# SamStudio8/gretel

Hardware: AMD Instinct MI355X
Metric: haplotypes/sec + SNP-edge-evals/sec on 10k-SNP synthetic contig (higher is better)
Workload: dtype f32 counts / f64 log-likelihoods

## Files before the change

gretel_amd/csrc/gretel_hip.hip:

```cpp

#include <hip/hip_runtime.h>

#include <algorithm>
#include <cmath>
#include <cstdarg>
#include <cstdio>
#include <cstdlib>
#include <cstring>
#include <atomic>
#include <chrono>
#include <map>
#include <mutex>
#include <new>
#include <string>
#include <thread>
#include <vector>

#include "gretel_hip.h"
#include "gh_detlog.h"


static thread_local char g_err[512] = "";

static int fail(int code, const char *fmt, ...)
// ... 1133 lines not shown
        return;
    }
    hipLaunchKernelGGL((k_scan<LC, false>), dim3(G1), dim3(SEG_THREADS), lds_scan, stream, P);
    hipLaunchKernelGGL((k_emit<LC>), dim3(S), dim3(SEG_THREADS), lds_emit, stream, P);
}

static int launch_seg_walk(gh_handle *h, uint8_t *d_path, double *d_lmsel, int rearm, int check_masks)
{
    int rc = alloc_seg(h);
    if (rc) return rc;
    seg_params P;
    P.N = h->N; P.L = h->L; P.rearm = rearm; P.check_masks = check_masks;
    P.G = h->lt; P.minfo = h->minfo; P.rinfo = h->rinfo; P.mt = h->cfg.marginal_term; P.nanp = h->cfg.marginal_term && h->cfg.offer_zero; P.sm = h->sm; P.st = h->dstate;
    P.hist = h->seg_hist; P.maps = h->seg_maps; P.pmaps = h->seg_pmaps; P.gmaps = h->seg_gmaps; P.segmin = h->seg_min;
    P.smin = h->seg_smin; P.gmin = h->seg_gmin; P.cm5snap = h->cm5snap;
    P.rws = 0; P.W = h->W; P.esz = (int)esize(h); P.band = h->band; P.halo = h->rws ? h->seg_halo : nullptr; P.patch_off = 0;
    P.rwflags = reinterpret_cast<int2 *>(h->seg_min + CW_MAX_SEG);
    P.path_out = d_path; P.lmsel = d_lmsel ? d_lmsel : h->lmsel1;
    if (h->L < 1 || h->L > SEG_MAX_L_NARROW) return fail(GH_ERR_STATE, "segment-parallel walk needs L <= %d", SEG_MAX_L_NARROW);
    prof_begin(h, GH_K_WALK);
    switch (h->L) {
        case 1: launch_seg_lc<1>(h, P); break;
        case 2: launch_seg_lc<2>(h, P); break;
        case 3: launch_seg_lc<3>(h, P); break;
        case 4: launch_seg_lc<4>(h, P); break;
        case 5: launch_seg_lc<5>(h, P); break;
        case 6: launch_seg_lc<6>(h, P); break;
    }
    prof_end(h, GH_K_WALK, (double)h->N * ((1.0 + (double)h->L) * CELL * esize(h) + 28.0));
    return post_launch(h, "k_seg/k_scan/k_emit");
}

static size_t rws_lds_bytes(int LC, bool five)
{
    (void)five;
    size_t b = max_cls(LC, [&](int R) { return seg_lds_total(R, LC); });
    if (b < (size_t)SEG_THREADS * 8) b = (size_t)SEG_THREADS * 8;
    return (b + 15) & ~(size_t)15;
}

static size_t rws_patch_off(const gh_handle *h, int LC)
{
    const bool five = seg_radix_ok(5, LC);
    const seg_geom g4 = seg_geometry(h->N, LC, 4), g5 = five ? seg_geometry(h->N, LC, 5) : g4;
    size_t off = rws_lds_bytes(LC, five);
    if (h->cfg.cond_mode == GH_COND_C || h->cfg.cond_mode == GH_COND_E) {
        const int longest = g4.seglen > g5.seglen ? g4.seglen : g5.seglen;
        const size_t need = (size_t)SEG_THREADS * 8 + (size_t)(longest + LC + 1) * NSYM * h->W * NSYM * esize(h);
        if (need > off) off = (need + 15) & ~(size_t)15;
    }
    return off;
}
#define RWS_LDS_MAX (160 * 1024 - 3 * 1024 - 512)

template <typename T, int LC, bool COL>
static void launch_rwseg_lc(gh_handle *h, seg_params P, const rws_params &Q)
{
    constexpr bool five = seg_radix_ok(5, LC);
    const int N = h->N;
    (void)five;
    const int S = (int)max_cls(LC, [&](int R) { return (size_t)seg_geometry(N, LC, R).S; }), G1 = (int)max_cls(LC, [&](int R) { return (size_t)seg_geometry(N, LC, R).G1; });
    const size_t off = rws_patch_off(h, LC);
    const size_t lds = off + sizeof(seg_patch);
    const size_t lds_scan = max_cls(LC, [&](int R) { return scan_lds_bytes(N, LC, R); });
    const size_t lds_emit = max_cls(LC, [&](int R) { return emit_lds_bytes(N, LC, R); });
    static std::atomic<size_t> set_rws[64], set_scan[64], set_emit[64];
    const int dv = h->dev & 63;
    if (lds > set_rws[dv]) { hipFuncSetAttribute((const void *)k_rwseg<T, LC, COL>, hipFuncAttributeMaxDynamicSharedMemorySize, (int)lds); set_rws[dv] = lds; }
    if (lds_scan > set_scan[dv]) { hipFuncSetAttribute((const void *)k_scan<LC, false>, hipFuncAttributeMaxDynamicSharedMemorySize, (int)lds_scan); set_scan[dv] = lds_scan; }
    if (lds_emit > set_emit[dv]) { hipFuncSetAttribute((const void *)k_emit<LC>, hipFuncAttributeMaxDynamicSharedMemorySize, (int)lds_emit); set_emit[dv] = lds_emit; }
    P.patch_off = (int)off;
    P.rws = 1;
    prof_begin(h, GH_K_RWSEG);
    hipLaunchKernelGGL((k_rwseg<T, LC, COL>), dim3(S), dim3(SEG_THREADS), lds, h->stream, P, Q);
    const int wl = h->W < LC ? h->W : LC;
    prof_end(h, GH_K_RWSEG, (double)N * (double)LC * CELL * esize(h) +
             (double)(N + 1) * ((double)h->W * 2.0 * esize(h) + 1.0 + CELL * esize(h) + 2 * 64 + 88 + 8) +
             (double)N * ((double)wl * 7 * esize(h) + (double)LC * LT_ROW * 8.0));
    const size_t lds_small = max_cls(LC, [&](int R) { return emit_small_lds_bytes(N, LC, R); });
    if (lds_small <= 64 * 1024 && !(getenv("GH_EMIT_SMALL") && atoi(getenv("GH_EMIT_SMALL")) == 0)) {
        static std::atomic<size_t> set_small[64];
        if (lds_small > set_small[dv]) { hipFuncSetAttribute((const void *)k_emit_small<LC>, hipFuncAttributeMaxDynamicSharedMemorySize, (int)lds_small); set_small[dv] = lds_small; }
        hipLaunchKernelGGL((k_emit_small<LC>), dim3(S), dim3(SEG_THREADS), lds_small, h->stream, P);
        return;
    }
    hipLaunchKernelGGL((k_scan<LC, false>), dim3(G1), dim3(SEG_THREADS), lds_scan, h->stream, P);
    hipLaunchKernelGGL((k_emit<LC>), dim3(S), dim3(SEG_THREADS), lds_emit, h->stream, P);
}

static int launch_rwseg(gh_handle *h, const uint8_t *d_prev, gh_path_rec *d_prev_rec, int prev_slot, double min_remove,
                        uint8_t *d_path, double *d_lmsel, int check_masks)
{
    int rc = alloc_seg(h);
    if (rc) return rc;
    seg_params P;
    P.N = h->N; P.L = h->L; P.rearm = 1; P.check_masks = check_masks;
    P.G = h->lt; P.minfo = h->minfo; P.rinfo = h->rinfo; P.mt = h->cfg.marginal_term; P.nanp = h->cfg.marginal_term && h->cfg.offer_zero; P.sm = h->sm; P.st = h->dstate;
    P.hist = h->seg_hist; P.maps = h->seg_maps; P.pmaps = h->seg_pmaps; P.gmaps = h->seg_gmaps; P.segmin = h->seg_min;
    P.smin = h->seg_smin; P.gmin = h->seg_gmin; P.cm5snap = h->cm5snap;
    P.rws = 1; P.W = h->W; P.esz = (int)esize(h); P.band = h->band; P.halo = h->seg_halo; P.patch_off = 0;
    P.rwflags = reinterpret_cast<int2 *>(h->seg_min + CW_MAX_SEG);
    P.path_out = d_path; P.lmsel = d_lmsel;
    rws_params Q;
    Q.band = h->band; Q.cnt = h->cnt; Q.marg = h->marg; Q.minfo = h->minfo; Q.rinfo = h->need_rinfo ? h->rinfo : nullptr; Q.G = h->lt;
    Q.nvalid = h->nvalid; Q.cmask = h->cmask; Q.path = d_prev; Q.min_remove = min_remove;
    Q.partial = h->partial + (size_t)prev_slot * h->spin_partial_stride;
    Q.rec = d_prev_rec; Q.cond_mode = h->cfg.cond_mode; Q.offer_zero = h->cfg.offer_zero;
    if (h->L < 1 || h->L > SEG_MAX_L_NARROW) return fail(GH_ERR_STATE, "k_rwseg needs L <= %d", SEG_MAX_L_NARROW);
    prof_begin(h, GH_K_WALK);
    const bool f64 = h->cfg.storage == GH_STORAGE_F64;
    const bool col = h->cfg.cond_mode == GH_COND_C || h->cfg.cond_mode == GH_COND_E;
    switch (h->L) {
#define RWS_CASE(n) case n: if (f64) { if (col) launch_rwseg_lc<double, n, true>(h, P, Q); else launch_rwseg_lc<double, n, false>(h, P, Q); } \
                            else { if (col) launch_rwseg_lc<float, n, true>(h, P, Q); else launch_rwseg_lc<float, n, false>(h, P, Q); } break;
        RWS_CASE(1) RWS_CASE(2) RWS_CASE(3) RWS_CASE(4) RWS_CASE(5) RWS_CASE(6)
#undef RWS_CASE
// ... 711 lines not shown
    *n_out = 0; *hole_at = 0;
    if (max_paths == 0) return GH_OK;
    int rc;
    if (!h->have_orig && (rc = gh_snapshot_original(h))) return rc;
    const size_t n1 = (size_t)h->N + 1;
    if ((rc = ensure_spin_buffers(h, max_paths))) return rc;
    uint8_t *d_paths = h->spin_paths;
    gh_path_rec *d_recs = h->spin_recs;
    hipError_t e = hipSuccess;
    rc = GH_OK;
    bool seg = seg_ok(h->wmode, h->L);
    h->seg6 = false;
    if (rc == GH_OK && !seg && h->wmode == WM_SEG && h->L == SEG_MAX_L_NARROW && !(getenv("GH_SEG6") && atoi(getenv("GH_SEG6")) == 0)) {
        rc = ensure_lt(h);
        dev_state look;
        if (rc == GH_OK) {
            e = hipMemcpyAsync(&look, h->dstate, sizeof look, hipMemcpyDeviceToHost, h->stream);
            if (e == hipSuccess) e = hipStreamSynchronize(h->stream);
            if (e != hipSuccess) rc = fail(GH_ERR_HIP, "gh_spin failed: %s", hipGetErrorString(e));
            else if (look.ranked) { seg = true; h->seg6 = true; }
        }
    }
    h->fuse = false;
    if (rc == GH_OK && seg && h->need_rinfo && h->W <= RW_FUSE_HALO && rw_lanes(h) == 8 && getenv("GH_FUSE") && atoi(getenv("GH_FUSE")) >= 1) {
        rc = ensure_lt(h);
        dev_state look;
        if (rc == GH_OK) {
            e = hipMemcpyAsync(&look, h->dstate, sizeof look, hipMemcpyDeviceToHost, h->stream);
            if (e == hipSuccess) e = hipStreamSynchronize(h->stream);
            if (e != hipSuccess) rc = fail(GH_ERR_HIP, "gh_spin failed: %s", hipGetErrorString(e));
            else {
                const int R = look.ranked ? 4 : 5;
                const int ppb = 256 / rw_lanes(h);
                const bool small = emit_small_lds_bytes(h->N, h->L, R) <= 64 * 1024 && !(getenv("GH_EMIT_SMALL") && atoi(getenv("GH_EMIT_SMALL")) == 0);
                const bool force = getenv("GH_FUSE") && atoi(getenv("GH_FUSE")) == 2;
                if ((!small || force) && seg_radix_ok(R, h->L) && rw_fuse_lds_bytes(h->N, h->L, R, ppb, h->W) <= 64 * 1024 && (rc = alloc_seg(h)) == GH_OK) {
                    h->fuse = true;
                    h->fuse_lds = rw_fuse_lds_bytes(h->N, h->L, R, ppb, h->W);
                    if (hipMemsetAsync(&h->dstate->maxstates, 0, sizeof(int), h->stream) != hipSuccess) rc = fail(GH_ERR_HIP, "gh_spin failed: hipMemsetAsync");
                }
            }
        }
    }
    h->rws = false;
    int rws_S = 0;
    if (rc == GH_OK && seg && !h->fuse && !h->lt_full && rw_lanes(h) == 8 &&
        !(getenv("GH_RWSEG") && atoi(getenv("GH_RWSEG")) == 0)) {
        const bool five = seg_radix_ok(5, h->L);
        const seg_geom g4 = seg_geometry(h->N, h->L, 4), g5 = five ? seg_geometry(h->N, h->L, 5) : g4;
        const bool small = (five ? max2(emit_small_lds_bytes(h->N, h->L, 4), emit_small_lds_bytes(h->N, h->L, 5)) : emit_small_lds_bytes(h->N, h->L, 4)) <= 64 * 1024 &&
                           !(getenv("GH_EMIT_SMALL") && atoi(getenv("GH_EMIT_SMALL")) == 0);
        const int longest = g4.seglen > g5.seglen ? g4.seglen : g5.seglen;
        const bool small_ok = !(getenv("GH_RWSEG_SMALL") && atoi(getenv("GH_RWSEG_SMALL")) == 0);
        if ((!small || small_ok) && longest + h->L + 1 <= SEG_THREADS / 8 && rws_patch_off(h, h->L) + sizeof(seg_patch) <= RWS_LDS_MAX &&
            (rc = alloc_seg(h)) == GH_OK) {
            rws_S = g4.S > g5.S ? g4.S : g5.S;
            const size_t need = (size_t)rws_S * h->L * NSYM * h->W * NSYM * esize(h);
            if (need > h->seg_halo_bytes) {
                if ((e = hipStreamSynchronize(h->stream)) != hipSuccess) rc = fail(GH_ERR_HIP, "gh_spin failed: %s", hipGetErrorString(e));
                else {
                    hipFree(h->seg_halo); h->seg_halo = nullptr; h->seg_halo_bytes = 0;
                    if (hipMalloc(&h->seg_halo, need) != hipSuccess) rc = fail(GH_ERR_NOMEM, "hipMalloc failed");
                    else h->seg_halo_bytes = need;
                }
            }
            h->rws = rc == GH_OK;
        }
    }
    int nb = rw_blocks(h, seg || cw_ok(h->wmode, h->L));
    if (h->rws && rws_S > nb) nb = rws_S;
    h->spin_partial_stride = nb;
    if (rc == GH_OK) rc = ensure_partial(h, nb, max_paths > h->spin_cap ? max_paths : h->spin_cap);
    if (rc == GH_OK) rc = reset_spin_state(h, h->rws ? h->partial : nullptr, h->rws ? (size_t)nb * max_paths : 0);
    const bool optimistic = seg && !h->lt_full;
    dev_state hs;
    memset(&hs, 0, sizeof hs);
    int first = 0;
    h->spin_requeues = 0;
    const bool cw = rc == GH_OK && !seg && cw_ok(h->wmode, h->L) && !h->cw_off;
    bool cw_gave_up = false;
    if (cw) {
        spin_io io;
        io.max_paths = max_paths; io.min_remove = min_remove; io.n1 = n1; io.nb = nb;
        io.d_paths = d_paths; io.d_recs = d_recs; io.paths_out = paths_out; io.recs = recs; io.no_reweight = false;
        rc = spin_candidate_pools(h, io, hs, &first, &cw_gave_up);
    }
    while ((!cw || cw_gave_up) && rc == GH_OK) {
        int launched = first;
        for (int s = first; s < max_paths && rc == GH_OK; s++) {
            if (!optimistic || s == first) { if ((rc = ensure_lt(h, !seg))) break; }
            const int cmk = !(optimistic && s > first) ? 0 : (s == h->force_stale_at && h->spin_requeues == 0 ? 2 : 1);
            if (h->rws) {
                if (s == first) rc = launch_walk(h, d_paths + n1 * s, d_recs + s, min_remove, 1, h->spin_lmsel + n1 * s, cmk);
                else rc = launch_rwseg(h, d_paths + n1 * (s - 1), d_recs + (s - 1), s - 1, min_remove, d_paths + n1 * s, h->spin_lmsel + n1 * s, cmk);
                if (rc == GH_OK && s == max_paths - 1)
                    rc = launch_reweight_marg(h, d_paths + n1 * s, min_remove, 1, d_recs + s, s, true, s > first, 0, h->spin_lmsel + n1 * s);
                if (rc) break;
                launched = s + 1;
                continue;
            }
            if ((rc = launch_walk(h, d_paths + n1 * s, d_recs + s, min_remove, 1, h->spin_lmsel + n1 * s, cmk))) break;
            if ((rc = launch_reweight_marg(h, d_paths + n1 * s, seg ? min_remove : 0.0, 1, d_recs + s, s, seg, optimistic && s > first, 0,
                                           h->spin_lmsel + n1 * s))) break;
            launched = s + 1;
        }
        if (rc == GH_OK && launched > 0 && (seg || cw_gave_up)) {
            hipLaunchKernelGGL(k_hp, dim3(launched, 2), dim3(64), 0, h->stream, (const double *)h->spin_lmsel, n1, (const uint8_t *)d_paths, n1,
// ... 1039 lines not shown
```

gretel_amd/csrc/segwalk.hpp:

```cpp
#pragma once

#include "seg_geom.hpp"

struct seg_params {
    int N, L;
    int rearm;
    int check_masks;
    const double *G;
    const double *minfo;
    const double *rinfo;
    int mt;
    int nanp;
    symmap sm;
    dev_state *st;
    uint32_t *hist;
    uint16_t *maps;
    uint16_t *pmaps;
    uint16_t *gmaps;
    double *segmin;
    double *smin;
    double *gmin;
    uint8_t *cm5snap;
    uint8_t *path_out;
    double *lmsel;
// ... 32 lines not shown
    if (first) {
        if (fr.x & 1) st->cm_same = 0;
        if (fr.x & 2) st->nodel = 0;
        if (fr.x & 4) st->narrow = 0;
        if (fr.y < st->first_hole) st->first_hole = fr.y;
    }
    if (P.check_masks == 2 || (P.check_masks && (fr.x & 1))) {
        if (first) st->lt_stale = 1;
        return false;
    }
    if (first) st->cur_hole = fr.y;
    return true;
}

template <int R>
__device__ __forceinline__ unsigned seg_argmax(const double (&vin)[R], bool nanp = false)
{
    static_assert(R == 4 || R == 5, "four ranks or five symbols");
    double v[R];
#pragma unroll
    for (int b = 0; b < R; b++) v[b] = vin[b];
    if (R == 5 && nanp) {
#pragma unroll
        for (int b = 1; b < R; b++) v[b] = v[b] != v[b] ? -INFINITY : v[b];
    }
    const bool c01 = v[1] > v[0], c23 = v[3] > v[2];
    const double m01 = vmax_f64(v[0], v[1]), m23 = vmax_f64(v[2], v[3]);
    const bool c = m23 > m01;
    unsigned idx = c ? (c23 ? 3u : 2u) : (c01 ? 1u : 0u);
    if constexpr (R == 5) {
        const double m = vmax_f64(m01, m23);
        idx = v[4] > m ? 4u : idx;
        idx = v[0] != v[0] ? 0u : idx;
    }
    return idx;
}

__device__ __forceinline__ double vmin_f64(double a, double b)
{
    double r;
    asm("v_min_f64 %0, %1, %2" : "=v"(r) : "v"(a), "v"(b));
    return r;
}

struct seg_patch {
    double row[SEG_MAX_L_NARROW][SEG_MAX_L_NARROW][LT_ROW];
    int row6[SEG_MAX_L_NARROW];
    int col[SEG_MAX_L_NARROW][SEG_MAX_L_NARROW];
    unsigned rmask[SEG_MAX_L_NARROW][SEG_MAX_L_NARROW];
    int colmode;
    double lm4[SEG_MAX_L_NARROW][4], lm5[SEG_MAX_L_NARROW][5];
    uint8_t cmall[SEG_THREADS / 8];
};

template <int R, int LC, bool TRACK, bool NANP = false>
__device__ __forceinline__ void seg_body(const seg_params &P, unsigned char *smem, const seg_patch *patch = nullptr)
{
    typedef typename seg_radix<R>::next_t next_t;
    constexpr int BITS = seg_radix<R>::BITS;
    constexpr unsigned MASK = (1u << BITS) - 1u;
    constexpr unsigned NS = seg_ipow(R, LC), NI = NS / R, RR = R * R;
    constexpr int CH = seg_chunk(R, LC);
    constexpr int SPT = (NS + SEG_THREADS - 1) / SEG_THREADS;
    const seg_geom g = seg_geometry(P.N, LC, R);
    const int s = blockIdx.x, tid = threadIdx.x;
    if (s >= g.S) return;
    const int t0 = s * g.seglen;
    const int t1 = t0 + g.seglen < P.N ? t0 + g.seglen : P.N;
    double *Gs = reinterpret_cast<double *>(smem);
    next_t *Nx = reinterpret_cast<next_t *>(Gs + (size_t)(CH + LC - 1) * LC * RR);
    double *Ms = reinterpret_cast<double *>(smem + seg_lds_bytes(R, LC));
    constexpr bool nanp = NANP;
    double mn[SPT];
#pragma unroll
    for (int q = 0; q < SPT; q++) mn[q] = INFINITY;

    unsigned sigma[SPT];
#pragma unroll
    for (int q = 0; q < SPT; q++) sigma[q] = (unsigned)(tid + q * SEG_THREADS) < NS ? (unsigned)(tid + q * SEG_THREADS) : 0u;

    SEG_STAMP(0);
    for (int c0 = t0; c0 < t1; c0 += CH) {
        const int nc = t1 - c0 < CH ? t1 - c0 : CH;
        const int nsrc = nc + LC - 1;
        for (int e = tid; e < nsrc * LC * R; e += SEG_THREADS) {
            const int d = e % R, l = (e / R) % LC, ii = e / (R * LC);
            const int i = c0 + 1 - LC + ii;
            double v[R];
#pragma unroll
            for (int b = 0; b < R; b++) v[b] = 0.0;
            if (i >= 0) {
                const double *src = P.G + (((size_t)i * 6 + (i == 0 ? 5 : d)) * LC + l) * LT_ROW;
#pragma unroll
                for (int b = 0; b < R; b++) v[b] = src[b];
                if (P.mt && l == 0) {
                    const double *lm = R == 4 ? P.rinfo + (size_t)(i + 1) * RINFO : P.minfo + (size_t)(i + 1) * MINFO;
                    if (patch && c0 == t0 && t0 > 0 && ii + 1 < LC) lm = R == 4 ? patch->lm4[ii + 1] : patch->lm5[ii + 1];
#pragma unroll
                    for (int b = 0; b < R; b++) v[b] = lm[b] + v[b];
                }
            }
            double *dst = Gs + (size_t)e * R;
#pragma unroll
            for (int b = 0; b < R; b++) dst[b] = v[b];
        }
        if (patch && c0 == t0 && t0 > 0) {
            __syncthreads();
            for (int e = tid; e < LC * LC * R; e += SEG_THREADS) {
                const int b = e % R, l = (e / R) % LC, hp = e / (R * LC);
                if (patch->colmode) {
                    const int col = patch->col[hp][l];
                    if (col >= 0 && col < R && ((patch->rmask[hp][l] >> b) & 1u)) {
                        double v = patch->row[hp][l][b];
                        if (P.mt && l == 0) {
                            const int i = t0 + 1 - LC + hp;
                            const double *lm = R == 4 ? P.rinfo + (size_t)(i + 1) * RINFO : P.minfo + (size_t)(i + 1) * MINFO;
                            if (hp + 1 < LC) lm = R == 4 ? patch->lm4[hp + 1] : patch->lm5[hp + 1];
                            v = lm[col] + v;
                        }
                        Gs[((size_t)(hp * LC + l) * R + b) * R + col] = v;
                    }
                    continue;
                }
                const int d = patch->row6[hp];
                if (d >= 0 && d < R) {
                    double v = patch->row[hp][l][b];
                    if (P.mt && l == 0) {
                        const int i = t0 + 1 - LC + hp;
                        const double *lm = R == 4 ? P.rinfo + (size_t)(i + 1) * RINFO : P.minfo + (size_t)(i + 1) * MINFO;
                        if (hp + 1 < LC) lm = R == 4 ? patch->lm4[hp + 1] : patch->lm5[hp + 1];
                        v = lm[b] + v;
                    }
                    Gs[((size_t)(hp * LC + l) * R + d) * R + b] = v;
                }
            }
        }
        if (TRACK) {
            for (int e = tid; e < nc * R; e += SEG_THREADS) {
                const int tl = e / R, b = e - tl * R;
                const int t = c0 + 1 + tl;
                Ms[e] = R == 4 ? P.rinfo[(size_t)t * RINFO + 4 + b] : P.minfo[(size_t)t * MINFO + 5 + b];
            }
        }
        __syncthreads();
        SEG_STAMP(1);
        {
            constexpr int SH = LC >= 4 ? 1 : 0;
            constexpr unsigned NJ = NI / (SH ? R : 1);
            for (unsigned task = tid; task < (unsigned)nc * NJ; task += SEG_THREADS) {
                const unsigned tl = task / NJ, j = task - tl * NJ;
                double xl[R][R];
#pragma unroll
                for (int dL = 0; dL < R; dL++) {
                    const double *row = Gs + ((size_t)(tl * LC + (LC - 1)) * R + dL) * R;
#pragma unroll
                    for (int b = 0; b < R; b++) xl[dL][b] = row[b];
                }
                double acc[R];
                unsigned rem = j;
                constexpr int NYOUNG = LC - 1 - SH;
                if constexpr (NYOUNG >= 1) {
#pragma unroll
                    for (int l = 1; l <= NYOUNG; l++) {
                        const unsigned d = rem % R;
                        rem /= R;
                        const double *row = Gs + ((size_t)((tl + LC - l) * LC + (l - 1)) * R + d) * R;
#pragma unroll
                        for (int b = 0; b < R; b++) acc[b] = l == 1 ? row[b] : acc[b] + row[b];
                    }
                }
#pragma unroll
                for (int dS = 0; dS < (SH ? R : 1); dS++) {
                    double acc2[R];
                    if constexpr (SH) {
                        const double *row = Gs + ((size_t)((tl + 1) * LC + (LC - 2)) * R + dS) * R;
#pragma unroll
                        for (int b = 0; b < R; b++) acc2[b] = NYOUNG >= 1 ? acc[b] + row[b] : row[b];
                    } else {
#pragma unroll
                        for (int b = 0; b < R; b++) acc2[b] = acc[b];
                    }
                    unsigned packed = 0;
#pragma unroll
                    for (int dL = 0; dL < R; dL++) {
                        double v[R];
#pragma unroll
                        for (int b = 0; b < R; b++) v[b] = LC >= 2 ? acc2[b] + xl[dL][b] : xl[dL][b];
                        packed |= seg_argmax<R>(v, nanp) << (BITS * dL);
                    }
                    Nx[(size_t)tl * NI + j + (SH ? dS * NJ : 0)] = (next_t)packed;
                }
            }
        }
        __syncthreads();
        SEG_STAMP(2);
        {
            constexpr int DPW = seg_radix<R>::DPW;
            const int w0 = (c0 - t0) / DPW;
            auto walk_word = [&](int tw, int nu, auto full_) {
                constexpr bool full = decltype(full_)::value;
                unsigned word[SPT];
#pragma unroll
                for (int q = 0; q < SPT; q++) word[q] = 0;
                const next_t *rows = Nx + (size_t)tw * NI;
#pragma unroll
                for (int u = 0; u < DPW; u++) {
                    if (full || u < nu) {
#pragma unroll
                        for (int q = 0; q < SPT; q++) {
                            const unsigned sg = sigma[q];
                            const unsigned hi = sg / NI, idx = sg - hi * NI;
                            const unsigned d = ((unsigned)rows[u * NI + idx] >> (BITS * hi)) & MASK;
                            word[q] |= d << (BITS * u);
                            sigma[q] = idx * R + d;
                            if (TRACK) mn[q] = vmin_f64(mn[q], Ms[(tw + u) * R + d]);
                        }
                    }
                }
#pragma unroll
                for (int q = 0; q < SPT; q++) {
                    const unsigned s0 = tid + q * SEG_THREADS;
                    if (s0 < NS) P.hist[((size_t)s * g.NW + w0 + tw / DPW) * NS + s0] = word[q];
                }
            };
            int tw = 0;
            for (; tw + DPW <= nc; tw += DPW) walk_word(tw, DPW, std::true_type{});
            if (tw < nc) walk_word(tw, nc - tw, std::false_type{});
        }
        SEG_STAMP(3);
        __syncthreads();
    }
#pragma unroll
    for (int q = 0; q < SPT; q++) {
        const unsigned s0 = tid + q * SEG_THREADS;
        if (s0 < NS) {
            P.maps[(size_t)s * NS + s0] = (uint16_t)sigma[q];
            if (TRACK) P.smin[(size_t)s * NS + s0] = mn[q];
        }
    }
    SEG_STAMP(4);
}

#include "segmix.hpp"

template <int LC, bool TRACK>
__global__ void __launch_bounds__(SEG_THREADS) k_seg(seg_params P)
{
    extern __shared__ __align__(16) unsigned char seg_smem[];
    dev_state *st = P.st;
    const dev_ctl c = load_ctl(st);
    if (c.stop || c.lt_stale) return;
    if (P.check_masks == 2 || (P.check_masks && c.cm_same == 0)) {
        if (blockIdx.x == 0 && threadIdx.x == 0) st->lt_stale = 1;
        return;
    }
    if (blockIdx.x == 0 && threadIdx.x == 0) st->cur_hole = c.first_hole;
    const int cls = __builtin_amdgcn_readfirstlane(seg_class(c, LC));
    if (cls == 4) seg_body<4, LC, TRACK>(P, seg_smem);
    else if constexpr (seg_radix_ok(5, LC)) {
        if constexpr (LC == SEGM_L && !TRACK) { if (cls == SEG_CLS_MIXED) { seg_body_mixed<LC, false>(P, seg_smem); return; } }
        if (P.nanp) seg_body<5, LC, TRACK, true>(P, seg_smem);
        else seg_body<5, LC, TRACK, false>(P, seg_smem);
    }
}

template <int R, int LC, bool TRACK>
__device__ __forceinline__ void scan_body(const seg_params &P, unsigned char *smem)
{
    constexpr int NS = seg_ns(R, LC);
    const seg_geom g = seg_geometry(P.N, LC, R);
    const int grp = blockIdx.x, tid = threadIdx.x;
    if (grp >= g.G1) return;
    const int s_lo = grp * g.G2;
    const int n = (s_lo + g.G2 <= g.S ? g.G2 : g.S - s_lo);
    uint16_t *M = reinterpret_cast<uint16_t *>(smem);
    const uint16_t *src = P.maps + (size_t)s_lo * NS;
    if constexpr (NS % 8 == 0) {
        const uint4 *s4 = reinterpret_cast<const uint4 *>(src);
        uint4 *d4 = reinterpret_cast<uint4 *>(M);
        for (int e = tid; e < n * (NS / 8); e += SEG_THREADS) d4[e] = s4[e];
    } else {
        for (int e = tid; e < n * NS; e += SEG_THREADS) M[e] = src[e];
// ... 787 lines not shown
    }
    RW_STAMP(4);
    __shared__ unsigned s_flags;
    __shared__ int s_hole;
    if (tid == 0) { s_flags = 0; s_hole = 0x7fffffff; }
#pragma unroll
    for (int o = 32; o > 0; o >>= 1) removed += __shfl_xor(removed, o);
    if ((tid & 63) == 0) s_sum4[tid >> 6] = removed;
    __syncthreads();
    if (flag_bits) atomicOr(&s_flags, flag_bits);
    if (hole_p != 0x7fffffff) atomicMin(&s_hole, hole_p);
    __syncthreads();
    if (tid == 0) {
        partial[blockIdx.x] = (s_sum4[0] + s_sum4[1]) + (s_sum4[2] + s_sum4[3]);
        const unsigned f = s_flags;
        if (f & 1u) atomicAnd(&st->cm_same, 0);
        if (f & 2u) atomicAnd(&st->nodel, 0);
        if (f & 4u) atomicAnd(&st->narrow, 0);
        if (s_hole != 0x7fffffff) atomicMin(&st->first_hole, s_hole);
    }
    RW_STAMP(5);
}

__device__ __forceinline__ double lane_f64(double v, int lane)
{
    const long long b = __double_as_longlong(v);
    const int lo = __builtin_amdgcn_readlane((int)b, lane), hi = __builtin_amdgcn_readlane((int)(b >> 32), lane);
    return __longlong_as_double(((long long)hi << 32) | (long long)(unsigned)lo);
}
__device__ __forceinline__ double wave_min_f64(double v)
{
    double x;
    x = dpp_f64<0xB1>(v); v = x < v ? x : v;
    x = dpp_f64<0x4E>(v); v = x < v ? x : v;
    x = dpp_f64<0x141>(v); v = x < v ? x : v;
    x = dpp_f64<0x140>(v); v = x < v ? x : v;
    const double r0 = lane_f64(v, 0), r1 = lane_f64(v, 16), r2 = lane_f64(v, 32), r3 = lane_f64(v, 48);
    const double a = r1 < r0 ? r1 : r0, b = r3 < r2 ? r3 : r2;
    return b < a ? b : a;
}

struct rws_params {
    void *band;
    double *cnt, *marg, *minfo, *rinfo, *G;
    int32_t *nvalid;
    uint32_t *cmask;
    const uint8_t *path;
    double min_remove;
    double *partial;
    gh_path_rec *rec;
    int cond_mode, offer_zero;
};

template <typename T, int LC, bool COL>
__device__ __forceinline__ bool rwseg_reweight(const seg_params &P, const rws_params &Q, const dev_ctl &c, unsigned char *smem, seg_patch *patch)
{
    const int N = P.N, W = P.W, L = LC, tid = threadIdx.x, sblk = blockIdx.x;
    const symmap sm = P.sm;
    dev_state *st = P.st;
    double *sred = reinterpret_cast<double *>(smem);
    __shared__ double s_logtab[256];
    logtab_stage(s_logtab);
    if (tid < SEG_MAX_L_NARROW) patch->row6[tid] = -1;
    if (tid < SEG_MAX_L_NARROW * SEG_MAX_L_NARROW) { (&patch->col[0][0])[tid] = -1; (&patch->rmask[0][0])[tid] = 0u; }
    if (tid == 0) patch->colmode = COL ? 1 : 0;
    const int R = seg_class(c, L);
    const seg_geom g = seg_geometry(N, L, R);
    if (sblk >= g.S) { if (tid == 0) { Q.partial[sblk] = 0.0; P.rwflags[sblk] = make_int2(0, 0x7fffffff); } return false; }
    RWS_STAMP(0);
    double vs[7];
#pragma unroll
    for (int k = 0; k < 7; k++) { const int q = (tid & 63) + 64 * k; vs[k] = q < g.S ? P.segmin[q] : INFINITY; }
    const int t0 = sblk * g.seglen;
    const int t1 = t0 + g.seglen < N ? t0 + g.seglen : N;
    const int nh = sblk > 0 ? L : 0;
    const int nown = (t1 - t0) + (sblk == 0 ? 1 : 0);
    const int slot = tid >> 3, s = tid & 7;
    const bool in = slot < nh + nown;
    const bool halo = in && slot < nh;
    const int p = !in ? 0 : (halo ? t0 + 1 - L + slot : (sblk == 0 ? slot : t0 + 1 + (slot - nh)));
    const bool act = in && p <= N;
    const bool own = act && !halo;
    const size_t pos_elems = (size_t)NSYM * W * NSYM;
    T *bandT = static_cast<T *>(Q.band);
    const T *blk = halo ? static_cast<const T *>(P.halo) + ((size_t)sblk * L + slot) * pos_elems : bandT + (size_t)p * pos_elems;
    if (COL) {
        T *blkL = reinterpret_cast<T *>(smem + (size_t)SEG_THREADS * 8);
        const size_t wper = pos_elems * sizeof(T) / 4;
        const uint32_t *srcH = reinterpret_cast<const uint32_t *>(static_cast<const T *>(P.halo) + (size_t)sblk * L * pos_elems);
        const int p_first = sblk == 0 ? 0 : t0 + 1;
        const uint32_t *srcO = reinterpret_cast<const uint32_t *>(bandT + (size_t)p_first * pos_elems);
        uint32_t *dst = reinterpret_cast<uint32_t *>(blkL);
        for (size_t q = tid; q < (size_t)nh * wper; q += SEG_THREADS) dst[q] = srcH[q];
        for (size_t q = tid; q < (size_t)nown * wper; q += SEG_THREADS) dst[(size_t)nh * wper + q] = srcO[q];
        __syncthreads();
        blk = blkL + (size_t)(in ? slot : 0) * pos_elems;
    }
    const int d0 = s + 1, j0 = p + d0;
    int mult0 = 0;
    if (act && d0 <= W) {
        if (j0 <= N - 1) mult0 = (d0 == 1) ? 2 : 1;
        else if (j0 == N) mult0 = (d0 == 1) ? 1 : 0;
        else if (j0 == N + 1) mult0 = (p == N) ? 1 : 0;
    }
    const int a = act ? Q.path[p] : 0;
    const int b0 = mult0 ? ((j0 == N + 1) ? Q.path[0] : Q.path[j0]) : 0;
    const bool lag_row = Q.G && act && p < N && d0 <= L && j0 <= N && (!COL || (mult0 > 0 && d0 <= W));
    T crow[NSYM];
#pragma unroll
    for (int x = 0; x < NSYM; x++) crow[x] = (act && s < NSYM) ? blk[((size_t)s * W) * NSYM + x] : (T)0;
    int nv_t = 0;
    uint32_t cm_t = 0;
    if (lag_row) { nv_t = Q.nvalid[j0]; cm_t = CM_CAND(Q.cmask[j0]); }
    const uint32_t cm_old = (own && s == 7) ? Q.cmask[p] : 0u;
    const bool need_row = act && d0 <= W && (mult0 > 0 || lag_row);
    const size_t roff = ((size_t)a * W + (size_t)((d0 <= W ? d0 : 1) - 1)) * NSYM;
    const size_t run0 = COL ? ((size_t)((d0 <= W ? d0 : 1) - 1)) * NSYM + b0 : roff;
    const size_t rstride = COL ? (size_t)W * NSYM : 1;
    const int esel = COL ? a : b0;
    T rrow[NSYM];
#pragma unroll
    for (int x = 0; x < NSYM; x++) rrow[x] = need_row ? blk[run0 + (size_t)x * rstride] : (T)0;
    double v0 = vs[0];
#pragma unroll
    for (int k = 1; k < 7; k++) v0 = vs[k] < v0 ? vs[k] : v0;
    const double minm = wave_min_f64(v0);
    RWS_STAMP(1);
    static_assert(SEG_MAX_L_NARROW * 8 <= 64 && SEG_MAX_L_NARROW * SEG_MAX_L_NARROW <= 64, "halo lane groups and the patch's arming lanes in one wavefront");
    const double ratio = minm < Q.min_remove ? Q.min_remove : minm;
    if (sblk == 0 && tid == 0) seg_finish(st, Q.rec, N, minm, Q.min_remove);
    RWS_STAMP(2);
    double removed = 0.0;
    int na = -1, nb = -1;
    T nval = (T)0;
    if (mult0) {
        T cur = rrow[0];
#pragma unroll
        for (int x = 1; x < NSYM; x++) cur = (x == esel) ? rrow[x] : cur;
        for (int q = 0; q < mult0; q++) {
            const double old = (double)cur;
            const double nw = old - ratio * old;
            cur = (T)nw;
            if (own) removed += old - nw;
        }
        if (own) bandT[(size_t)p * pos_elems + roff + b0] = cur;
#pragma unroll
        for (int x = 0; x < NSYM; x++) rrow[x] = (x == esel) ? cur : rrow[x];
        if (d0 == 1) { na = a; nb = b0; nval = cur; }
    }
    na = __shfl(na, 0, 8); nb = __shfl(nb, 0, 8);
    nval = (T)__shfl((double)nval, 0, 8);
    __syncthreads();
    unsigned flag_bits = 0;
    int hole_p = 0x7fffffff;
    double cs[NSYM];
    double tot = 0.0;
    int nv = 0;
    uint32_t cm = 0;
    T acc = (T)0;
#pragma unroll
    for (int x = 0; x < NSYM; x++) {
        T v = crow[x];
        if (s == na && x == nb) v = nval;
        acc = acc + v;
    }
    const double mine = (double)acc;
#pragma unroll
    for (int x = 0; x < NSYM; x++) {
        cs[x] = __shfl(mine, x, 8);
        if (cs[x] > 0) {
            tot += cs[x];
            if ((VALID_MASK >> x) & 1) { nv++; cm |= 1u << x; }
        }
    }
    const uint32_t cand = Q.offer_zero ? VALID_MASK : cm;
    const uint32_t cmw = cm | (cand << 8);
    const uint32_t cm5 = cm5_of_cmask(sm, cand);
    if (own) {
        if (s < NSYM) {
// ... 92 lines not shown
        const double nv_i = (double)nv;
        int row6 = a6;
        if (ranked && a6 < 5) row6 = ((cm5 >> a6) & 1u) ? __popc(cm5 & ((1u << a6) - 1u)) : -1;
        if (row6 >= 0) {
            double out[LT_ROW];
            if (!(a6 < 5 || p == 0)) {
#pragma unroll
                for (int q = 0; q < LT_ROW; q++) out[q] = 0.0;
            } else {
                double rowv[NSYM];
                T racc = (T)0;
#pragma unroll
                for (int x = 0; x < NSYM; x++) { rowv[x] = (double)rrow[x]; racc = racc + rrow[x]; }
                const double sum = (double)racc;
                const double den = (Q.cond_mode == GH_COND_A) ? (double)nv_t + sum : (Q.cond_mode == GH_COND_D ? nv_i + sum : nv_i + ca);
                constexpr int VS[LT_ROW] = {0, 1, 2, 3, 5};
                double xq[LT_ROW], v[LT_ROW];
                bool odd = false;
#pragma unroll
                for (int q = 0; q < LT_ROW; q++) xq[q] = (1.0 + rowv[VS[q]]) / den;
#pragma unroll
                for (int q = 0; q < LT_ROW; q++) odd |= !gh_log10_is_normal(xq[q]);
#pragma unroll
                for (int q = 0; q < LT_ROW; q++) v[q] = gh_log10_normal_tab(xq[q], 0, s_logtab, GH_LOG_BOTH);
                if (odd) {
#pragma unroll
                    for (int q = 0; q < LT_ROW; q++) v[q] = gh_log10_tab(xq[q], s_logtab, GH_LOG_BOTH);
                }
#pragma unroll
                for (int q = 0; q < LT_ROW; q++) out[q] = -INFINITY;
                if (!ranked) {
#pragma unroll
                    for (int q = 0; q < LT_ROW; q++) {
                        const int b5 = a6_of_sym(sm, VS[q]);
                        const double val = ((cm_t >> VS[q]) & 1) ? v[q] : -INFINITY;
#pragma unroll
                        for (int w = 0; w < LT_ROW; w++) out[w] = (b5 == w) ? val : out[w];
                    }
                } else {
                    const uint32_t cj5 = cm5_of_cmask(sm, cm_t);
#pragma unroll
                    for (int q = 0; q < LT_ROW; q++) {
                        const int b5 = a6_of_sym(sm, VS[q]);
                        const int rb = ((cj5 >> b5) & 1u) ? __popc(cj5 & ((1u << b5) - 1u)) : -1;
#pragma unroll
                        for (int w = 0; w < LT_ROW; w++) out[w] = (rb == w) ? v[q] : out[w];
                    }
                }
            }
            if (own) {
                double *dst = Q.G + (((size_t)p * 6 + row6) * L + (d0 - 1)) * LT_ROW;
#pragma unroll
                for (int q = 0; q < LT_ROW; q++) dst[q] = out[q];
            } else {
#pragma unroll
                for (int q = 0; q < LT_ROW; q++) patch->row[slot][d0 - 1][q] = out[q];
                if (s == 0) patch->row6[slot] = row6;
            }
        }
    }
    RWS_STAMP(4);
    __shared__ unsigned s_flags;
    __shared__ int s_hole;
    __shared__ double s_part[32];
    if (tid == 0) { s_flags = 0; s_hole = 0x7fffffff; }
    sred[tid] = removed;
    __syncthreads();
    if (flag_bits) atomicOr(&s_flags, flag_bits);
    if (hole_p != 0x7fffffff) atomicMin(&s_hole, hole_p);
    if (tid < 32) {
        const int nact = 8 * (nh + nown);
        double a2 = 0.0;
        for (int q = tid; q < nact; q += 32) a2 += sred[q];
        s_part[tid] = a2;
    }
    __syncthreads();
    if (tid == 0) {
        double tot_removed = 0.0;
#pragma unroll
        for (int q = 0; q < 32; q++) tot_removed += s_part[q];
        Q.partial[sblk] = tot_removed;
        const unsigned f = s_flags;
        if (f & 1u) atomicAnd(&st->cm_same, 0);
        if (f & 2u) atomicAnd(&st->nodel, 0);
        if (f & 4u) atomicAnd(&st->narrow, 0);
        if (s_hole != 0x7fffffff) atomicMin(&st->first_hole, s_hole);
        P.rwflags[sblk] = make_int2((int)f, s_hole);
    }
    __threadfence_block();
    __syncthreads();
    RWS_STAMP(5);
    return true;
}

template <typename T, int LC, bool COL>
__global__ void __launch_bounds__(SEG_THREADS) k_rwseg(seg_params P, rws_params Q)
{
    extern __shared__ __align__(16) unsigned char seg_smem[];
    dev_state *st = P.st;
    const dev_ctl c = load_ctl(st);
    if (c.stop || c.lt_stale || c.cw_unres) return;
    if (c.cur_hole <= P.N) {
        if (blockIdx.x == 0 && threadIdx.x == 0) seg_finish(st, Q.rec, P.N, 0.0, Q.min_remove);
        return;
    }
    seg_patch *patch = reinterpret_cast<seg_patch *>(seg_smem + P.patch_off);
    if (!rwseg_reweight<T, LC, COL>(P, Q, c, seg_smem, patch)) return;
    const int cls = __builtin_amdgcn_readfirstlane(seg_class(c, LC));
    if (cls == 4) seg_body<4, LC, false>(P, seg_smem, patch);
    else if constexpr (seg_radix_ok(5, LC)) {
        if constexpr (LC == SEGM_L) { if (cls == SEG_CLS_MIXED) { seg_body_mixed<LC, true>(P, seg_smem, patch); return; } }
        if (P.nanp) seg_body<5, LC, false, true>(P, seg_smem, patch);
        else seg_body<5, LC, false, false>(P, seg_smem, patch);
    }
}

__global__ void __launch_bounds__(256) k_seg_fin(seg_params P, gh_path_rec *rec, double min_remove, int nseg_arg)
{
    __shared__ double s_red[256];
    dev_state *st = P.st;
    if (st->stop || st->lt_stale || st->cw_unres) return;
    const int nseg = nseg_arg > 0 ? nseg_arg : seg_count(st, P.N, P.L);
    double mine = INFINITY;
    for (int q = threadIdx.x; q < nseg; q += 256) {
        const double v = P.segmin[q];
        if (v < mine) mine = v;
    }
    s_red[threadIdx.x] = mine;
    __syncthreads();
    for (int q = 128; q > 0; q >>= 1) {
        if ((int)threadIdx.x < q && s_red[threadIdx.x + q] < s_red[threadIdx.x]) s_red[threadIdx.x] = s_red[threadIdx.x + q];
        __syncthreads();
    }
    if (threadIdx.x == 0) seg_finish(st, rec, P.N, s_red[0], min_remove);
}

#define HP_CHUNK 512
template <int WHICH>
__device__ __forceinline__ double hp_sum(const double *lm, const uint8_t *path, const double *minfo, int N, double (*buf)[HP_CHUNK], symmap sm)
{
    const int lane = threadIdx.x;
    auto value = [&](int t) -> double {
        const int tt = t <= N ? t : N;
        const double v = WHICH == 0 ? lm[tt] : minfo[(size_t)tt * MINFO + 11 + a6_of_sym(sm, path[tt])];
        return t <= N ? v : 0.0;
    };
    constexpr int PER = HP_CHUNK / 64;
    double r[PER];
#pragma unroll
    for (int k = 0; k < PER; k++) r[k] = value(1 + lane + 64 * k);
    const int nchunks = (N + HP_CHUNK - 1) / HP_CHUNK;
    double acc = 0.0;
    for (int c = 0; c < nchunks; c++) {
        double *b = buf[c & 1];
#pragma unroll
        for (int k = 0; k < PER; k++) b[lane + 64 * k] = r[k];
        __syncthreads();
        if (c + 1 < nchunks) {
#pragma unroll
            for (int k = 0; k < PER; k++) r[k] = value(1 + (c + 1) * HP_CHUNK + lane + 64 * k);
        }
#pragma unroll 32
        for (int j = 0; j < HP_CHUNK; j++) acc += b[j];
    }
    return acc;
}
// ... 18 lines not shown
```

Measured before the change: 29570.

## Prefetch first segment slice into LDS asynchronously during reweight phase

The fused reweight+segment kernel now issues asynchronous global-to-LDS loads (global_load_lds) for the first chunk of the G table while the reweight phase is still computing. Rows the reweight rewrites are also patched into that LDS copy, so seg_body can skip its initial staging loop. The reduction scratch moves past the patch so it does not clash with the prefetched slice. Some __syncthreads are replaced with lighter LDS-only fence+barrier sequences. This hides global load latency but costs extra LDS, adds complexity, and relies on ordering between rewritten rows and the async copy.

```diff
diff --git a/gretel_amd/csrc/gretel_hip.hip b/gretel_amd/csrc/gretel_hip.hip
--- a/gretel_amd/csrc/gretel_hip.hip
+++ b/gretel_amd/csrc/gretel_hip.hip
@@ -1209,6 +1209,12 @@
     return off;
 }
 #define RWS_LDS_MAX (160 * 1024 - 3 * 1024 - 512)
+static size_t rws_lds_need(const gh_handle *h, int LC)
+{
+    const size_t off = rws_patch_off(h, LC);
+    if (h->cfg.cond_mode == GH_COND_C || h->cfg.cond_mode == GH_COND_E) return off + sizeof(seg_patch);
+    return rws_sred_off(off) + (size_t)SEG_THREADS * 8;
+}
 
 template <typename T, int LC, bool COL>
 static void launch_rwseg_lc(gh_handle *h, seg_params P, const rws_params &Q)
@@ -1218,7 +1224,7 @@
     (void)five;
     const int S = (int)max_cls(LC, [&](int R) { return (size_t)seg_geometry(N, LC, R).S; }), G1 = (int)max_cls(LC, [&](int R) { return (size_t)seg_geometry(N, LC, R).G1; });
     const size_t off = rws_patch_off(h, LC);
-    const size_t lds = off + sizeof(seg_patch);
+    const size_t lds = rws_lds_need(h, LC);
     const size_t lds_scan = max_cls(LC, [&](int R) { return scan_lds_bytes(N, LC, R); });
     const size_t lds_emit = max_cls(LC, [&](int R) { return emit_lds_bytes(N, LC, R); });
     static std::atomic<size_t> set_rws[64], set_scan[64], set_emit[64];
@@ -2036,7 +2042,7 @@
                            !(getenv("GH_EMIT_SMALL") && atoi(getenv("GH_EMIT_SMALL")) == 0);
         const int longest = g4.seglen > g5.seglen ? g4.seglen : g5.seglen;
         const bool small_ok = !(getenv("GH_RWSEG_SMALL") && atoi(getenv("GH_RWSEG_SMALL")) == 0);
-        if ((!small || small_ok) && longest + h->L + 1 <= SEG_THREADS / 8 && rws_patch_off(h, h->L) + sizeof(seg_patch) <= RWS_LDS_MAX &&
+        if ((!small || small_ok) && longest + h->L + 1 <= SEG_THREADS / 8 && rws_lds_need(h, h->L) <= RWS_LDS_MAX &&
             (rc = alloc_seg(h)) == GH_OK) {
             rws_S = g4.S > g5.S ? g4.S : g5.S;
             const size_t need = (size_t)rws_S * h->L * NSYM * h->W * NSYM * esize(h);
diff --git a/gretel_amd/csrc/segwalk.hpp b/gretel_amd/csrc/segwalk.hpp
--- a/gretel_amd/csrc/segwalk.hpp
+++ b/gretel_amd/csrc/segwalk.hpp
@@ -108,9 +108,17 @@
     double lm4[SEG_MAX_L_NARROW][4], lm5[SEG_MAX_L_NARROW][5];
     uint8_t cmall[SEG_THREADS / 8];
 };
+__host__ __device__ constexpr size_t rws_sred_off(size_t patch_off) { return (patch_off + sizeof(seg_patch) + 15) & ~(size_t)15; }
+
+__device__ __forceinline__ void lds_barrier()
+{
+    __builtin_amdgcn_fence(__ATOMIC_RELEASE, "workgroup", "local");
+    __builtin_amdgcn_s_barrier();
+    __builtin_amdgcn_fence(__ATOMIC_ACQUIRE, "workgroup", "local");
+}
 
 template <int R, int LC, bool TRACK, bool NANP = false>
-__device__ __forceinline__ void seg_body(const seg_params &P, unsigned char *smem, const seg_patch *patch = nullptr)
+__device__ __forceinline__ void seg_body(const seg_params &P, unsigned char *smem, const seg_patch *patch = nullptr, bool pre = false)
 {
     typedef typename seg_radix<R>::next_t next_t;
     constexpr int BITS = seg_radix<R>::BITS;
@@ -139,7 +147,8 @@
     for (int c0 = t0; c0 < t1; c0 += CH) {
         const int nc = t1 - c0 < CH ? t1 - c0 : CH;
         const int nsrc = nc + LC - 1;
-        for (int e = tid; e < nsrc * LC * R; e += SEG_THREADS) {
+        const bool pre0 = pre && c0 == t0;
+        if (!pre0) for (int e = tid; e < nsrc * LC * R; e += SEG_THREADS) {
             const int d = e % R, l = (e / R) % LC, ii = e / (R * LC);
             const int i = c0 + 1 - LC + ii;
             double v[R];
@@ -161,7 +170,7 @@
             for (int b = 0; b < R; b++) dst[b] = v[b];
         }
         if (patch && c0 == t0 && t0 > 0) {
-            __syncthreads();
+            if (!pre0) __syncthreads();
             for (int e = tid; e < LC * LC * R; e += SEG_THREADS) {
                 const int b = e % R, l = (e / R) % LC, hp = e / (R * LC);
                 if (patch->colmode) {
@@ -198,7 +207,8 @@
                 Ms[e] = R == 4 ? P.rinfo[(size_t)t * RINFO + 4 + b] : P.minfo[(size_t)t * MINFO + 5 + b];
             }
         }
-        __syncthreads();
+        if (pre0) lds_barrier();
+        else __syncthreads();
         SEG_STAMP(1);
         {
             constexpr int SH = LC >= 4 ? 1 : 0;
@@ -284,6 +294,7 @@
             if (tw < nc) walk_word(tw, nc - tw, std::false_type{});
         }
         SEG_STAMP(3);
+        if (pre0 && c0 + CH < t1) __threadfence_block();
         __syncthreads();
     }
 #pragma unroll
@@ -1177,13 +1188,36 @@
     int cond_mode, offer_zero;
 };
 
+template <int R, int LC>
+__device__ __forceinline__ void rws_slice_issue(const double *G, unsigned char *smem, int t0, int nsrc)
+{
+    constexpr int RR = R * R;
+    const int ndw = nsrc * LC * RR * 2;
+    const int lane = threadIdx.x & 63;
+    uint32_t *dst = reinterpret_cast<uint32_t *>(smem);
+    const uint32_t *src = reinterpret_cast<const uint32_t *>(G);
+    for (int q0 = __builtin_amdgcn_readfirstlane((int)threadIdx.x >> 6) * 64; q0 < ndw; q0 += SEG_THREADS) {
+        const int q = q0 + lane;
+        if (q >= ndw) break;
+        const int e = q >> 1, b = e % R, d = (e / R) % R, l = (e / RR) % LC, ii = e / (RR * LC);
+        const int i = t0 + 1 - LC + ii;
+        if (i >= 0) {
+            const size_t w = ((((size_t)i * 6 + (i == 0 ? 5 : d)) * LC + l) * LT_ROW + b) * 2 + (q & 1);
+            __builtin_amdgcn_global_load_lds(src + w, (__attribute__((address_space(3))) void *)(dst + q0), 4, 0, 0);
+        } else {
+            dst[q] = 0u;
+        }
+    }
+}
+
 template <typename T, int LC, bool COL>
-__device__ __forceinline__ bool rwseg_reweight(const seg_params &P, const rws_params &Q, const dev_ctl &c, unsigned char *smem, seg_patch *patch)
+__device__ __forceinline__ bool rwseg_reweight(const seg_params &P, const rws_params &Q, const dev_ctl &c, unsigned char *smem, seg_patch *patch,
+                                               bool &pre)
 {
     const int N = P.N, W = P.W, L = LC, tid = threadIdx.x, sblk = blockIdx.x;
     const symmap sm = P.sm;
     dev_state *st = P.st;
-    double *sred = reinterpret_cast<double *>(smem);
+    double *sred = reinterpret_cast<double *>(COL ? smem : smem + rws_sred_off(P.patch_off));
     __shared__ double s_logtab[256];
     logtab_stage(s_logtab);
     if (tid < SEG_MAX_L_NARROW) patch->row6[tid] = -1;
@@ -1191,6 +1225,7 @@
     if (tid == 0) patch->colmode = COL ? 1 : 0;
     const int R = seg_class(c, L);
     const seg_geom g = seg_geometry(N, L, R);
+    pre = !COL && !P.mt && (R == 4 || (R == 5 && seg_radix_ok(5, LC)));
     if (sblk >= g.S) { if (tid == 0) { Q.partial[sblk] = 0.0; P.rwflags[sblk] = make_int2(0, 0x7fffffff); } return false; }
     RWS_STAMP(0);
     double vs[7];
@@ -1228,16 +1263,19 @@
         else if (j0 == N) mult0 = (d0 == 1) ? 1 : 0;
         else if (j0 == N + 1) mult0 = (p == N) ? 1 : 0;
     }
-    const int a = act ? Q.path[p] : 0;
-    const int b0 = mult0 ? ((j0 == N + 1) ? Q.path[0] : Q.path[j0]) : 0;
+    const int pa = Q.path[act ? p : 0], pb = Q.path[(mult0 && j0 <= N) ? j0 : 0];
+    const int a = act ? pa : 0;
+    const int b0 = mult0 ? pb : 0;
     const bool lag_row = Q.G && act && p < N && d0 <= L && j0 <= N && (!COL || (mult0 > 0 && d0 <= W));
     T crow[NSYM];
 #pragma unroll
     for (int x = 0; x < NSYM; x++) crow[x] = (act && s < NSYM) ? blk[((size_t)s * W) * NSYM + x] : (T)0;
-    int nv_t = 0;
-    uint32_t cm_t = 0;
-    if (lag_row) { nv_t = Q.nvalid[j0]; cm_t = CM_CAND(Q.cmask[j0]); }
-    const uint32_t cm_old = (own && s == 7) ? Q.cmask[p] : 0u;
+    const int jt = lag_row ? j0 : 0;
+    const int nv_l = Q.nvalid[jt];
+    const uint32_t cm_l = Q.cmask[jt], cm_p = Q.cmask[own ? p : 0];
+    const int nv_t = lag_row ? nv_l : 0;
+    const uint32_t cm_t = lag_row ? CM_CAND(cm_l) : 0u;
+    const uint32_t cm_old = (own && s == 7) ? cm_p : 0u;
     const bool need_row = act && d0 <= W && (mult0 > 0 || lag_row);
     const size_t roff = ((size_t)a * W + (size_t)((d0 <= W ? d0 : 1) - 1)) * NSYM;
     const size_t run0 = COL ? ((size_t)((d0 <= W ? d0 : 1) - 1)) * NSYM + b0 : roff;
@@ -1246,10 +1284,16 @@
     T rrow[NSYM];
 #pragma unroll
     for (int x = 0; x < NSYM; x++) rrow[x] = need_row ? blk[run0 + (size_t)x * rstride] : (T)0;
+    const int nsrc0 = (t1 - t0 < seg_chunk(R, L) ? t1 - t0 : seg_chunk(R, L)) + L - 1;
+    if (pre) {
+        if (R == 4) rws_slice_issue<4, LC>(P.G, smem, t0, nsrc0);
+        else if constexpr (seg_radix_ok(5, LC)) rws_slice_issue<5, LC>(P.G, smem, t0, nsrc0);
+    }
     double v0 = vs[0];
 #pragma unroll
     for (int k = 1; k < 7; k++) v0 = vs[k] < v0 ? vs[k] : v0;
     const double minm = wave_min_f64(v0);
+    if (pre) __builtin_amdgcn_s_waitcnt(0x0F70);
     RWS_STAMP(1);
     static_assert(SEG_MAX_L_NARROW * 8 <= 64 && SEG_MAX_L_NARROW * SEG_MAX_L_NARROW <= 64, "halo lane groups and the patch's arming lanes in one wavefront");
     const double ratio = minm < Q.min_remove ? Q.min_remove : minm;
@@ -1448,6 +1492,15 @@
                 double *dst = Q.G + (((size_t)p * 6 + row6) * L + (d0 - 1)) * LT_ROW;
 #pragma unroll
                 for (int q = 0; q < LT_ROW; q++) dst[q] = out[q];
+                const int ii = p - (t0 + 1 - L);
+                if (pre && ii < nsrc0) {
+                    double *gs = reinterpret_cast<double *>(smem) + (size_t)(ii * L + (d0 - 1)) * R * R;
+                    for (int d = 0; d < R; d++) {
+                        if (p == 0 ? row6 != 5 : row6 != d) continue;
+#pragma unroll
+                        for (int q = 0; q < LT_ROW; q++) if (q < R) gs[d * R + q] = out[q];
+                    }
+                }
             } else {
 #pragma unroll
                 for (int q = 0; q < LT_ROW; q++) patch->row[slot][d0 - 1][q] = out[q];
@@ -1483,8 +1536,12 @@
         if (s_hole != 0x7fffffff) atomicMin(&st->first_hole, s_hole);
         P.rwflags[sblk] = make_int2((int)f, s_hole);
     }
-    __threadfence_block();
-    __syncthreads();
+    if (pre) {
+        lds_barrier();
+    } else {
+        __threadfence_block();
+        __syncthreads();
+    }
     RWS_STAMP(5);
     return true;
 }
@@ -1501,13 +1558,14 @@
         return;
     }
     seg_patch *patch = reinterpret_cast<seg_patch *>(seg_smem + P.patch_off);
-    if (!rwseg_reweight<T, LC, COL>(P, Q, c, seg_smem, patch)) return;
+    bool pre = false;
+    if (!rwseg_reweight<T, LC, COL>(P, Q, c, seg_smem, patch, pre)) return;
     const int cls = __builtin_amdgcn_readfirstlane(seg_class(c, LC));
-    if (cls == 4) seg_body<4, LC, false>(P, seg_smem, patch);
+    if (cls == 4) seg_body<4, LC, false>(P, seg_smem, patch, pre);
     else if constexpr (seg_radix_ok(5, LC)) {
         if constexpr (LC == SEGM_L) { if (cls == SEG_CLS_MIXED) { seg_body_mixed<LC, true>(P, seg_smem, patch); return; } }
-        if (P.nanp) seg_body<5, LC, false, true>(P, seg_smem, patch);
-        else seg_body<5, LC, false, false>(P, seg_smem, patch);
+        if (P.nanp) seg_body<5, LC, false, true>(P, seg_smem, patch, pre);
+        else seg_body<5, LC, false, false>(P, seg_smem, patch, pre);
     }
 }
 
```

After: 27280 (median of 2 runs). 0.923x the previous value.
